# facebookresearch/SlowFast

Measured on AMD Instinct MI355X. Metric: clips/sec (fwd+bwd), SlowFast-8x8-R50 32x224^2 synthetic clips, per-GPU batch 32, higher is better.
Workload: dtype fp16; 1 GPU; SLOWFAST_8x8_R50: forward + cross_entropy loss + backward + sgd step, inputs resident in HBM, per-GPU batch 32; global_batch=32, parallelism=dp1, launch=hip-graph(fwd+bwd) + eager all-reduce/optimizer, optimizer=FlatOptimizer (fused unscale+norm+clip+update, dynamic loss scale on device)

## Files before the change

### slowfast_amd/csrc/sf_api.hip

```cpp
#include "../../include/sfamd.h"
#include "sf_bn.h"
#include "sf_common.h"
#include "sf_igemm.h"
#include "sf_igemm2.h"
#include "sf_wgrad2.h"
#include "sf_pool.h"
#include "sf_dwconv.h"
#include "sf_dwsweep.h"
#include "sf_dwtemporal.h"
#include "sf_tokens.h"
#include "sf_x3d.h"
#include "sf_stem.h"
#include "sf_attn.h"
#include "sf_roi.h"
#include "sf_optim.h"

#include <stdarg.h>
#include <stdio.h>
#include <stdlib.h>
#include <string.h>

static thread_local char g_err[512] = "";

static int fail(const char* fmt, ...) {
// ... 466 lines not shown
    memset(&p, 0, sizeof(p));
    p.g = gather_fwd(d, x, in_scale, in_shift, in_relu);
    p.M = d->N * d->To * d->Ho * d->Wo;
    int32_t ldf, ldd;
    sf_conv_weight_ld(d, &ldf, &ldd);
    p.wmat = (const f16*)wf; p.ldw = ldf; p.Nout = d->Co;
    p.ksteps = cdiv(p.g.Ktot, 32);
    p.y = (f16*)y; p.ldy = d->ldy;
    p.bias = bias; p.resid = nullptr; p.ldr = 0;
    p.stat_part = stat_part;
    return run_igemm(p, is_pointwise(d), (hipStream_t)stream);
}

extern "C" int sf_conv_fwd_fused(const sf_conv_desc* d, const void* x, const void* wf, const float* bias,
                                 const void* resid, int32_t ldr, int out_relu, void* y, sf_stream_t stream) {
    if (check_desc(d)) return -1;
    REQUIRE(x && wf && y, "sf_conv_fwd_fused: null pointer");
    REQUIRE(!resid || (ldr >= d->Co && ldr % 8 == 0), "sf_conv_fwd_fused: bad residual pitch");
    if (!resid) {
        const StemPlan sp = plan_stem(d);
        if (sp.ok) {
            StemParams q = stem_params(d, sp, x);
            int32_t ldf0, ldd0;
            sf_conv_weight_ld(d, &ldf0, &ldd0);
            q.wmat = (const f16*)wf; q.ldw = ldf0; q.y = (f16*)y;
            q.bias = bias; q.out_relu = out_relu;
            SF_STEM_FWD_LAUNCH(sp, q, stream);
            return check_launch("stem_fwd_fused");
        }
    }
    IgemmParams p;
    memset(&p, 0, sizeof(p));
    p.g = gather_fwd(d, x, nullptr, nullptr, 0);
    p.M = d->N * d->To * d->Ho * d->Wo;
    int32_t ldf, ldd;
    sf_conv_weight_ld(d, &ldf, &ldd);
    p.wmat = (const f16*)wf; p.ldw = ldf; p.Nout = d->Co;
    p.ksteps = cdiv(p.g.Ktot, 32);
    p.y = (f16*)y; p.ldy = d->ldy;
    p.bias = bias; p.resid = (const f16*)resid; p.ldr = ldr;
    p.act_mode = out_relu ? 3 : 0;
    return run_igemm(p, is_pointwise(d), (hipStream_t)stream);
}

struct BnFuse {
    const float* scale; const float* shift; const void* bits;
    const void* y0; int32_t ld0; float* part0;
};
static int conv_dgrad_impl(const sf_conv_desc* d, const void* dy, const void* wd, const void* resid, int32_t ldr,
                           const void* resid_bits, void* dx, const BnFuse* bn, int32_t* bn_rows, sf_stream_t stream) {
    if (check_desc(d)) return -1;
    REQUIRE(dy && wd && dx, "sf_conv_dgrad: null pointer");
    REQUIRE(!resid || (ldr >= d->Ci && ldr % 8 == 0), "sf_conv_dgrad: bad residual pitch");
    IgemmParams p;
    memset(&p, 0, sizeof(p));
    p.g = gather_dgrad(d, dy);
    p.M = d->N * d->Ti * d->Hi * d->Wi;
    int32_t ldf, ldd;
    sf_conv_weight_ld(d, &ldf, &ldd);
    p.wmat = (const f16*)wd; p.ldw = ldd; p.Nout = d->Ci;
    p.ksteps = cdiv(p.g.Ktot, 32);
    p.y = (f16*)dx; p.ldy = d->ldx;
    p.resid = (const f16*)resid; p.ldr = ldr;
    REQUIRE(!resid_bits || resid, "sf_conv_dgrad: resid_bits without a residual");
    p.resid_bits = (const uint8_t*)resid_bits;
    const bool fuse = bn && d->sT == 1 && d->sH == 1 && d->sW == 1;
    if (!resid && d->Co == 8 && d->To == d->Ti && d->Ho == d->Hi && d->Wo == d->Wi) {
        sf_conv_desc dd = *d;
        dd.Ci = d->Co; dd.Cw = d->Co; dd.Co = d->Ci; dd.Cow = 0;
        dd.pT = d->kT - 1 - d->pT; dd.pH = d->kH - 1 - d->pH; dd.pW = d->kW - 1 - d->pW;
        dd.ldx = d->ldy; dd.ldy = d->ldx;
        const StemPlan sp = plan_stem(&dd);
        if (sp.ok && sp.thin3 && (!fuse || sp.ntiles <= cdiv(p.M, 128))) {
            StemParams q = stem_params(&dd, sp, dy);
            const int S = d->kT * d->kH;
            q.wmat = (const f16*)wd; q.ldw = ldd; q.y = (f16*)dx;
            q.wo0 = ((S - 1) * 3 + 2) * 8; q.wos = -24; q.wog = -8; q.kwc = 3;
            if (fuse) {
                q.bnb_y = (const f16*)bn->y0; q.bnb_ld = bn->ld0; q.bnb_scale = bn->scale; q.bnb_shift = bn->shift;
                q.bnb_bits = (const uint8_t*)bn->bits;
                q.stat_part = bn->part0; q.stat_rows = 0;
            }
            SF_STEM_FWD_LAUNCH(sp, q, stream);
            if (bn_rows) *bn_rows = fuse ? sp.ntiles : 0;
            return check_launch("stem_dgrad");
        }
    }
    if (fuse) {
        p.bnb_y = (const f16*)bn->y0; p.bnb_ld = bn->ld0; p.bnb_part = bn->part0;
        p.bnb_scale = bn->scale; p.bnb_shift = bn->shift; p.bnb_bits = (const uint8_t*)bn->bits;
    }
    int bm = 0;
    const int rc = run_igemm(p, is_pointwise(d), (hipStream_t)stream, &bm);
    if (bn_rows) *bn_rows = (fuse && bm > 0) ? cdiv(p.M, bm) : 0;
    return rc;
}

extern "C" int sf_conv_dgrad(const sf_conv_desc* d, const void* dy, const void* wd, const void* resid, int32_t ldr,
                             const void* resid_bits, void* dx, sf_stream_t stream) {
    return conv_dgrad_impl(d, dy, wd, resid, ldr, resid_bits, dx, nullptr, nullptr, stream);
}

extern "C" int sf_conv_dgrad_bn(const sf_conv_desc* d, const void* dy, const void* wd, const void* resid, int32_t ldr,
                                const void* resid_bits, void* dx, const float* mask_scale, const float* mask_shift,
                                const void* mask_bits, const void* bn_y, int32_t bn_ldy, float* bn_part, int32_t bn_part_rows,
                                int32_t* bn_rows, sf_stream_t stream) {
    REQUIRE(d && bn_y && bn_part && bn_rows, "sf_conv_dgrad_bn: null pointer");
    REQUIRE(mask_bits || (mask_scale && mask_shift), "sf_conv_dgrad_bn: a mask source is needed (mask_bits, or mask_scale + mask_shift)");
    REQUIRE(bn_ldy >= d->Ci && bn_ldy % 8 == 0 && ((uintptr_t)bn_y & 15) == 0, "sf_conv_dgrad_bn: bad bn_y pitch / alignment");
    REQUIRE((int64_t)bn_part_rows * 128 >= (int64_t)d->N * d->Ti * d->Hi * d->Wi,
            "sf_conv_dgrad_bn: the partial table needs ceil(positions / 128) rows of [2][Ci] floats");
    const BnFuse bn = {mask_scale, mask_shift, mask_bits, bn_y, bn_ldy, bn_part};
    return conv_dgrad_impl(d, dy, wd, resid, ldr, resid_bits, dx, &bn, bn_rows, stream);
}

template <int BMW, int WM, int WN, int KS>
static void launch_wgrad(WgradParams& p, dim3 grid3, hipStream_t s) {
    p.tiles_k = grid3.x; p.tiles_c = grid3.y;
    const dim3 grid(grid3.x * grid3.y * grid3.z);
    hipLaunchKernelGGL((sf_wgrad_kernel<BMW, WM, WN, KS>), grid, dim3(SF_THREADS), 0, s, p);
}

struct WgradPlan {
    int BMW, KS, tiles_k, tiles_c, Co_pad, Kpad, nchunks, chunks_per_split, splits;
    size_t ws_bytes;
};
static WgradPlan plan_wgrad(const sf_conv_desc* d) {
    WgradPlan w;
    const int taps = d->kT * d->kH * d->kW;
    const int Ktot = taps * d->Ci;
    const int64_t M = (int64_t)d->N * d->To * d->Ho * d->Wo;
    w.BMW = d->Co >= 128 ? 128 : d->Co >= 64 ? 64 : d->Co >= 32 ? 32 : 16;
    w.KS = w.BMW <= 32 ? 4 : 1;
    w.tiles_k = cdiv(Ktot, 128);
    w.tiles_c = cdiv(d->Co, w.BMW);
    w.Kpad = w.tiles_k * 128;
    w.Co_pad = w.tiles_c * w.BMW;
    w.nchunks = cdiv(M, 32);
    const int64_t slab = (int64_t)w.Co_pad * w.Kpad * 4;
    static const int target = tune_knob("SF_WGRAD_BLOCKS", 1024);
    int splits = cdiv(target, (int64_t)w.tiles_k * w.tiles_c);
    const int64_t cap = (256ll << 20) / slab;
    if (splits > cap) splits = (int)(cap < 1 ? 1 : cap);
    const int nstages = cdiv(w.nchunks, w.KS);
    if (splits > nstages) splits = nstages;
    if (splits < 1) splits = 1;
    w.chunks_per_split = cdiv(nstages, splits) * w.KS;
    w.splits = cdiv(w.nchunks, w.chunks_per_split);
    w.ws_bytes = (size_t)slab * w.splits;
    return w;
}

struct Wgrad2Plan {
    bool ok, thin, dual;
    int BMW, BKW, tiles_k, tiles_c, Co_pad, Kpad, rows_per_split, splits;
    int slabs;
    size_t tab_bytes, ws_bytes;
};
static Wgrad2Plan plan_wgrad2(const sf_conv_desc* d) {
    Wgrad2Plan w;
    memset(&w, 0, sizeof(w));
    const char* e;
    if (test_hook("SF_WGRAD2", 1) == 0) return w;
    const int mink = test_hook("SF_WGRAD2_MINK", 192);
    const int minrows = test_hook("SF_WGRAD2_MINROWS", 4096);
    const int taps = d->kT * d->kH * d->kW;
    const int target = test_hook("SF_WGRAD2_BLOCKS", 512);
    (void)taps;
    const int Ktot = taps * d->Ci;
    const int64_t M = (int64_t)d->N * d->To * d->Ho * d->Wo;
    if (taps > SF_I2_MAXTAPS || M < minrows) return w;
    if ((d->kT - 1) * d->dT > 127 || (d->kH - 1) * d->dH > 127 || (d->kW - 1) * d->dW > 127) return w;
    if (plan_stem(d).ok) return w;
    if (d->Co <= 32) {
        if (test_hook("SF_WGRAD2T", 1) == 0) return w;
        const int minrows_t = test_hook("SF_WGRAD2T_MINROWS", 16384);
        if (M < minrows_t) return w;
        w.thin = true;
        w.BMW = d->Co <= 16 ? 16 : 32;
        w.BKW = Ktot <= 32 ? 32 : 128;
        w.tiles_k = cdiv(Ktot, w.BKW);
        w.tiles_c = 1;
        w.Kpad = w.tiles_k * w.BKW;
        w.Co_pad = w.BMW;
        const int target_t = test_hook("SF_WGRAD2T_BLOCKS", w.BKW == 128 ? 512 : w.BMW == 32 ? 768 : 1024);
        int splits = target_t / w.tiles_k;
        if (splits < 1) splits = 1;
        w.rows_per_split = roundup(cdiv(M, splits), 128);
        w.splits = cdiv(M, w.rows_per_split);
        w.tab_bytes = ((size_t)M * 8 + 255) / 256 * 256 + 1280;
        w.ws_bytes = w.tab_bytes + (size_t)w.Co_pad * w.Kpad * 4 * w.splits;
        w.slabs = w.splits;
        w.ok = true;
        return w;
    }
    if (Ktot < mink) return w;
    w.BMW = d->Co > 64 ? 128 : 64;
    w.tiles_k = cdiv(Ktot, 256);
    w.tiles_c = cdiv(d->Co, w.BMW);
    w.Kpad = w.tiles_k * 256;
    w.Co_pad = w.tiles_c * w.BMW;
    int splits = target / (w.tiles_k * w.tiles_c);
    const int64_t slab = (int64_t)w.Co_pad * w.Kpad * 4;
    const int64_t cap = (256ll << 20) / slab;
    if (splits > cap) splits = (int)(cap < 1 ? 1 : cap);
    if (splits < 1) splits = 1;
    w.dual = false;
    if (splits >= 2 && test_hook("SF_WGRAD2_DUAL", 1) != 0) {
        const int tiles = w.tiles_k * w.tiles_c;
        const int pairs = (target / 2) / tiles;
        const int64_t steps = cdiv(cdiv(M, splits), 32);
        if (pairs >= 1 && 2 * pairs * 10 >= (2 * pairs < splits ? splits : 2 * pairs) * 9 && steps <= test_hook("SF_WGRAD2_DUAL_STEPS", 80)) {
            w.dual = true;
            if (2 * pairs < splits) splits = 2 * pairs;
        }
    }
    w.rows_per_split = roundup(cdiv(M, splits), 32);
    w.splits = cdiv(M, w.rows_per_split);
    if (w.splits < 2) w.dual = false;
    w.slabs = w.dual ? cdiv(w.splits, 2) : w.splits;
    w.tab_bytes = ((size_t)M * 8 + 255) / 256 * 256 + 1280;
    w.ws_bytes = w.tab_bytes + (size_t)slab * w.splits;
    w.ok = true;
    return w;
}

static void launch_rowtab(const sf_conv_desc* d, void* tab, hipStream_t s) {
    RowtabParams t;
    memset(&t, 0, sizeof(t));
    t.tab = (i32x2*)tab;
    t.M = d->N * d->To * d->Ho * d->Wo;
    t.fdW = make_fastdiv(d->Wo); t.fdH = make_fastdiv(d->Ho); t.fdT = make_fastdiv(d->To);
    t.sT = d->Ti; t.sH = d->Hi; t.sW = d->Wi;
    t.strT = d->sT; t.strH = d->sH; t.strW = d->sW; t.padT = d->pT; t.padH = d->pH; t.padW = d->pW;
    t.ntaps = d->kT * d->kH * d->kW;
    int ti = 0;
    for (int kt = 0; kt < d->kT; ++kt)
        for (int kh = 0; kh < d->kH; ++kh)
            for (int kw = 0; kw < d->kW; ++kw, ++ti) {
                t.dt[ti] = (int8_t)(kt * d->dT); t.dh[ti] = (int8_t)(kh * d->dH); t.dw[ti] = (int8_t)(kw * d->dW);
            }
    hipLaunchKernelGGL(sf_wgrad2_rowtab_kernel, dim3(cdiv(t.M, SF_THREADS)), dim3(SF_THREADS), 0, s, t);
}

extern "C" int64_t sf_conv_wgrad_rowtab_bytes(const sf_conv_desc* d) {
    if (check_desc(d)) return -1;
    const Wgrad2Plan w2 = plan_wgrad2(d);
    return w2.ok ? (int64_t)w2.tab_bytes : 0;
}

extern "C" int sf_conv_wgrad_rowtab(const sf_conv_desc* d, void* tab, sf_stream_t stream) {
    if (check_desc(d)) return -1;
    REQUIRE(tab && (uintptr_t)tab % 16 == 0, "sf_conv_wgrad_rowtab: tab must be a 16-byte aligned device pointer");
    REQUIRE(plan_wgrad2(d).ok, "sf_conv_wgrad_rowtab: this geometry does not take the row-table kernel (sf_conv_wgrad_rowtab_bytes == 0)");
    launch_rowtab(d, tab, (hipStream_t)stream);
    return check_launch("wgrad_rowtab");
}

extern "C" int64_t sf_conv_wgrad_workspace(const sf_conv_desc* d) {
    if (check_desc(d)) return -1;
    int64_t generic = (int64_t)plan_wgrad(d).ws_bytes;
    const Wgrad2Plan w2 = plan_wgrad2(d);
    if (w2.ok && (int64_t)w2.ws_bytes > generic) generic = (int64_t)w2.ws_bytes;
    const StemPlan sp = plan_stem(d);
    return sp.ok && (int64_t)sp.ws_bytes > generic ? (int64_t)sp.ws_bytes : generic;
}

extern "C" int sf_conv_wgrad(const sf_conv_desc* d, const void* x, const float* in_scale, const float* in_shift,
                             int in_relu, const void* dy, float* dw, float out_scale, int zero_first,
                             void* workspace, int64_t workspace_bytes, const void* rowtab, sf_stream_t stream) {
    if (check_desc(d)) return -1;
    REQUIRE(x && dy && dw && workspace, "sf_conv_wgrad: null pointer");
    REQUIRE((in_scale == nullptr) == (in_shift == nullptr), "sf_conv_wgrad: in_scale/in_shift must come together");
    REQUIRE(!in_scale || d->Ci <= 512, "sf_conv_wgrad: fused input BatchNorm supports Ci <= 512 (got %d)", d->Ci);
    hipStream_t s = (hipStream_t)stream;
    int splits, Co_pad, Kpad;
    GatherSide gk = gather_fwd(d, x, in_scale, in_shift, in_relu);
    const StemPlan sp = plan_stem(d);
    const Wgrad2Plan w2 = in_scale ? Wgrad2Plan{} : plan_wgrad2(d);
    float* slabs = (float*)workspace;
    if (w2.ok) {
        REQUIRE(workspace_bytes >= (int64_t)w2.ws_bytes, "sf_conv_wgrad: workspace too small (%lld < %lld bytes)",
                (long long)workspace_bytes, (long long)w2.ws_bytes);
        REQUIRE(((uintptr_t)x | (uintptr_t)dy | (uintptr_t)workspace) % 16 == 0, "sf_conv_wgrad: operands must be 16-byte aligned");
        Wgrad2Params q;
        memset(&q, 0, sizeof(q));
        int ti = 0;
        for (int kt = 0; kt < d->kT; ++kt)
            for (int kh = 0; kh < d->kH; ++kh)
                for (int kw = 0; kw < d->kW; ++kw, ++ti) q.dlin[ti] = (kt * d->dT * d->Hi + kh * d->dH) * d->Wi + kw * d->dW;
        if (!rowtab) launch_rowtab(d, workspace, s);
        else REQUIRE((uintptr_t)rowtab % 16 == 0, "sf_conv_wgrad: rowtab must be 16-byte aligned");
        q.x = (const f16*)x; q.ldx = d->ldx; q.C = d->Ci;
        q.dy = (const f16*)dy; q.ldy = d->ldy; q.Co = d->Co;
        q.M = d->N * d->To * d->Ho * d->Wo; q.Ktot = gk.Ktot;
        q.rowtab = (const i32x2*)(rowtab ? rowtab : workspace);
        slabs = (float*)((char*)workspace + w2.tab_bytes);
        q.ws = slabs; q.Co_pad = w2.Co_pad; q.Kpad = w2.Kpad;
        q.tiles_k = w2.tiles_k; q.tiles_c = w2.tiles_c; q.rows_per_split = w2.rows_per_split;
        q.stage_stride = (w2.thin && tune_knob("SF_WGRAD2T_RR", 1) != 0) ? w2.splits : 0;
        const dim3 grid((unsigned)(w2.tiles_k * w2.tiles_c * w2.slabs));
        static const bool trace = test_hook("SF_TRACE", 0) != 0;
        if (trace) fprintf(stderr, "[sfamd] wgrad2: M=%d Co=%d K=%d tiles %dx%d splits %d%s\n", q.M, q.Co, q.Ktot, w2.tiles_c, w2.tiles_k, w2.splits,
                           w2.dual ? " (two per workgroup)" : "");
        if (w2.thin) {
            if (w2.BMW == 16 && w2.BKW == 128) hipLaunchKernelGGL((sf_wgrad2t_kernel<16, 128, 2>), grid, dim3(256), 0, s, q);
            else if (w2.BMW == 32 && w2.BKW == 128) hipLaunchKernelGGL((sf_wgrad2t_kernel<32, 128, 2>), grid, dim3(256), 0, s, q);
            else if (w2.BMW == 16) hipLaunchKernelGGL((sf_wgrad2t_kernel<16, 32, 3>), grid, dim3(256), 0, s, q);
            else hipLaunchKernelGGL((sf_wgrad2t_kernel<32, 32, 3>), grid, dim3(256), 0, s, q);
        } else if (w2.dual) {
            if (w2.BMW == 128) hipLaunchKernelGGL((sf_wgrad2_kernel<128, true>), grid, dim3(1024), 0, s, q);
            else hipLaunchKernelGGL((sf_wgrad2_kernel<64, true>), grid, dim3(1024), 0, s, q);
        } else {
            if (w2.BMW == 128) hipLaunchKernelGGL((sf_wgrad2_kernel<128>), grid, dim3(512), 0, s, q);
            else hipLaunchKernelGGL((sf_wgrad2_kernel<64>), grid, dim3(512), 0, s, q);
        }
        splits = w2.slabs; Co_pad = w2.Co_pad; Kpad = w2.Kpad;
    } else if (sp.ok && !in_scale) {
        REQUIRE(workspace_bytes >= (int64_t)sp.ws_bytes, "sf_conv_wgrad: workspace too small (%lld < %lld bytes)",
                (long long)workspace_bytes, (long long)sp.ws_bytes);
        StemParams q = stem_params(d, sp, x);
        q.dy = (const f16*)dy; q.ws = (float*)workspace;
        const bool trace = test_hook("SF_TRACE", 0) != 0;
        if (trace) fprintf(stderr, "[sfamd] stem_wgrad: %d workgroups x %d tiles\n", sp.wg_blocks, sp.tiles_per_block);
        static const bool stem_plain = tune_knob("SF_STEM_XCD", 1) == 0;
        q.plain_order = stem_plain ? 1 : 0;
        if (d->Co <= 8 && sp.small) hipLaunchKernelGGL((sf_stem_wgrad_kernel<8, SF_STEM_CHUNKS_SMALL>), dim3(sp.wg_blocks), dim3(SF_STEM_WG_THREADS), 0, s, q);
        else if (d->Co <= 8) hipLaunchKernelGGL((sf_stem_wgrad_kernel<8, SF_STEM_CHUNKS>), dim3(sp.wg_blocks), dim3(SF_STEM_WG_THREADS), 0, s, q);
        else if (sp.small) hipLaunchKernelGGL((sf_stem_wgrad_kernel<16, SF_STEM_CHUNKS_SMALL>), dim3(sp.wg_blocks), dim3(SF_STEM_WG_THREADS), 0, s, q);
        else hipLaunchKernelGGL((sf_stem_wgrad_kernel<16, SF_STEM_CHUNKS>), dim3(sp.wg_blocks), dim3(SF_STEM_WG_THREADS), 0, s, q);
        splits = sp.wg_blocks * sp.wgroups; Co_pad = 16; Kpad = sp.Kpad;
    } else {
        const WgradPlan w = plan_wgrad(d);
        REQUIRE(workspace_bytes >= (int64_t)w.ws_bytes, "sf_conv_wgrad: workspace too small (%lld < %lld bytes)",
                (long long)workspace_bytes, (long long)w.ws_bytes);
        REQUIRE(w.splits <= 65535, "sf_conv_wgrad: too many splits");
        WgradParams p;
        memset(&p, 0, sizeof(p));
        p.g = gk;
        p.dy = (const f16*)dy; p.ldy = d->ldy; p.Co = d->Co;
        p.M = d->N * d->To * d->Ho * d->Wo;
        p.ws = (float*)workspace; p.Co_pad = w.Co_pad; p.Kpad = w.Kpad;
        p.nchunks = w.nchunks; p.chunks_per_split = w.chunks_per_split;
        dim3 grid(w.tiles_k, w.tiles_c, w.splits);
        switch (w.BMW) {
            case 128: launch_wgrad<128, 64, 64, 1>(p, grid, s); break;
            case 64: launch_wgrad<64, 32, 64, 1>(p, grid, s); break;
            case 32: launch_wgrad<32, 32, 32, 4>(p, grid, s); break;
            default: launch_wgrad<16, 16, 32, 4>(p, grid, s); break;
        }
        splits = w.splits; Co_pad = w.Co_pad; Kpad = w.Kpad;
    }
    if (check_launch("wgrad")) return -1;
    WgradReduceParams r;
    r.ws = slabs; r.splits = splits; r.Co = d->Cow ? d->Cow : d->Co; r.Co_pad = Co_pad; r.Kpad = Kpad;
    r.Ktot = gk.Ktot; r.fdC = gk.fdC; r.dw = dw; r.Cw = d->Cw; r.taps = d->kT * d->kH * d->kW;
    r.slice4 = 0;
    if (sp.ok && sp.thin3 && !in_scale && !w2.ok) { r.slice4 = 1; r.Ktot = d->kT * d->kH * 32; }
    r.out_scale = out_scale; r.accumulate = zero_first ? 0 : 1;
    int64_t total = (int64_t)r.Co * Kpad / 4;
    int lanes = 1;
    while (lanes < 32 && lanes * 4 <= splits) lanes *= 2;
    r.lanes = lanes;
    const int per_block = SF_THREADS / lanes;
    hipLaunchKernelGGL(sf_wgrad_reduce_kernel, dim3(cdiv(total, per_block)), dim3(SF_THREADS), 0, s, r);
    return check_launch("wgrad_reduce");
}

static RowTile make_rowtile(int64_t M, int C, int max_blocks, dim3& grid) {
    RowTile rt;
    rt.M = (int)M; rt.C = C;
    const int G = C / 8;
    const int TG = G < SF_THREADS ? G : SF_THREADS;
    const int rpi = SF_THREADS / TG;
    int passes = cdiv(M, (int64_t)rpi * max_blocks);
    if (passes < 1) passes = 1;
    rt.rows_per_block = rpi * passes;
    grid = dim3(cdiv(M, rt.rows_per_block), cdiv(G, SF_THREADS));
    return rt;
}
static int check_rows(const char* who, int64_t M, int C) {
    REQUIRE(M > 0 && M < (1ll << 31), "%s: bad row count", who);
    REQUIRE(C > 0 && C % 8 == 0, "%s: C must be a positive multiple of 8 (got %d)", who, C);
    return 0;
}

static const int kFoldAbove = tune_knob("SF_FOLD_ABOVE", 2048);
static int fold_partials(float* part, int& nblk, int C, hipStream_t s) {
    if (nblk <= kFoldAbove || nblk <= 256) return 1;
    const int group = nblk <= 2048 ? 16 : nblk <= 8192 ? 32 : 64;
    const int cols = 2 * C;
    dim3 grid(cdiv(cols, SF_THREADS), cdiv(nblk, group));
    hipLaunchKernelGGL(sf_part_fold_kernel, grid, dim3(SF_THREADS), 0, s, part, nblk, cols, group);
    nblk = cdiv(nblk, group);
    return group;
}

extern "C" int sf_bn_finalize(float* part, int32_t nblk, int32_t C, int32_t Creal, float count, const float* gamma,
                              const float* beta, float* running_mean, float* running_var, float momentum, float eps,
                              float* scale, float* shift, float* save_mean, float* save_rstd, sf_stream_t stream) {
    REQUIRE(gamma && beta && scale && shift, "sf_bn_finalize: null pointer");
    REQUIRE(nblk > 0 ? part != nullptr : (running_mean && running_var), "sf_bn_finalize: missing statistics source");
    REQUIRE(Creal > 0 && Creal <= C, "sf_bn_finalize: Creal must be in (0, C]");
    BnFinalizeParams p;
    p.row_stride = nblk > 0 ? fold_partials(part, nblk, C, (hipStream_t)stream) : 1;
    p.part = part; p.nblk = nblk; p.C = C; p.Creal = Creal; p.count = count; p.gamma = gamma; p.beta = beta;
    p.running_mean = running_mean; p.running_var = running_var; p.momentum = momentum; p.eps = eps;
    p.scale = scale; p.shift = shift; p.save_mean = save_mean; p.save_rstd = save_rstd;
    hipLaunchKernelGGL(sf_bn_finalize_kernel, dim3(cdiv(C, SF_FIN_CH)), dim3(sf_fin_threads(p.nblk)), 0, (hipStream_t)stream, p);
    return check_launch("bn_finalize");
}

extern "C" int sf_bn_act(int64_t M, int32_t C, const void* y, int32_t ldy, const float* scale, const float* shift,
                         const void* r, int32_t ldr, const float* rscale, const float* rshift, int relu, void* out,
                         int32_t ldo, void* mask_out, sf_stream_t stream) {
    if (check_rows("sf_bn_act", M, C)) return -1;
    REQUIRE(y && out, "sf_bn_act: null pointer");
    BnActParams p;
    dim3 grid;
    p.rt = make_rowtile(M, C, 8192, grid);
    p.y = (const f16*)y; p.ldy = ldy; p.scale = scale; p.shift = shift;
    p.r = (const f16*)r; p.ldr = ldr; p.rscale = rscale; p.rshift = rshift;
    p.relu = relu; p.out = (f16*)out; p.ldo = ldo; p.mask_out = (uint8_t*)mask_out;
    hipLaunchKernelGGL(sf_bn_act_kernel, grid, dim3(SF_THREADS), 0, (hipStream_t)stream, p);
    return check_launch("bn_act");
}

static const int kBwdBlocks = tune_knob("SF_BN_BWD_BLOCKS", 1024);
extern "C" int sf_bn_bwd_blocks(int64_t M, int32_t C) {
    if (check_rows("sf_bn_bwd_blocks", M, C)) return -1;
    dim3 grid;
    make_rowtile(M, C, kBwdBlocks, grid);
    return (int)grid.x;
}

extern "C" int sf_bn_bwd_reduce(int64_t M, int32_t C, const void* dz, int32_t lddz, const void* zmask, int32_t ldm,
                                const void* y, int32_t ldy, const float* scale, const float* shift, int relu_self,
                                float* part, sf_stream_t stream) {
    if (check_rows("sf_bn_bwd_reduce", M, C)) return -1;
    REQUIRE(dz && y && part, "sf_bn_bwd_reduce: null pointer");
    REQUIRE(!relu_self || (scale && shift), "sf_bn_bwd_reduce: relu_self needs scale/shift");
    BnBwdReduceParams p;
    dim3 grid;
    p.rt = make_rowtile(M, C, kBwdBlocks, grid);
    p.dz = (const f16*)dz; p.lddz = lddz; p.zmask = (const f16*)zmask; p.ldm = ldm;
    p.y = (const f16*)y; p.ldy = ldy; p.scale = scale; p.shift = shift; p.relu_self = relu_self; p.part = part;
    hipLaunchKernelGGL(sf_bn_bwd_reduce_kernel, grid, dim3(SF_THREADS), 0, (hipStream_t)stream, p);
    return check_launch("bn_bwd_reduce");
}

extern "C" int sf_bn_bwd_finalize(float* part, int32_t nblk, int32_t C, int32_t Creal, float count, const float* gamma,
                                  const float* mean, const float* rstd, float inv_loss_scale, float* dgamma,
                                  float* dbeta, int accumulate, float* coef, sf_stream_t stream) {
    REQUIRE(part && gamma && mean && rstd && dgamma && dbeta && coef, "sf_bn_bwd_finalize: null pointer");
    BnBwdFinalizeParams p;
    p.row_stride = fold_partials(part, nblk, C, (hipStream_t)stream);
    REQUIRE(Creal > 0 && Creal <= C, "sf_bn_bwd_finalize: Creal must be in (0, C]");
    p.part = part; p.nblk = nblk; p.C = C; p.Creal = Creal; p.count = count; p.gamma = gamma; p.mean = mean; p.rstd = rstd;
    p.inv_loss_scale = inv_loss_scale; p.dgamma = dgamma; p.dbeta = dbeta; p.accumulate = accumulate; p.coef = coef;
    hipLaunchKernelGGL(sf_bn_bwd_finalize_kernel, dim3(cdiv(C, SF_FIN_CH)), dim3(sf_fin_threads(p.nblk)), 0, (hipStream_t)stream, p);
    return check_launch("bn_bwd_finalize");
}
// ... 1632 lines not shown
```

### slowfast_amd/csrc/sf_wgrad2.h

```cpp
#pragma once
#include "sf_common.h"
#include "sf_igemm2.h"

struct __attribute__((aligned(8))) i32x2 { int32_t x, y; };
typedef int32_t i32x8 __attribute__((ext_vector_type(8)));

struct Wgrad2Params {
    const f16* x; int ldx, C;
    const f16* dy; int ldy, Co;
    int M;
    int Ktot;
    const i32x2* rowtab;
    int32_t dlin[SF_I2_MAXTAPS];
    float* ws;
    int Co_pad, Kpad;
    int tiles_k, tiles_c;
    int rows_per_split;
    int stage_stride;
};

struct RowtabParams {
    i32x2* tab;
    int M;
    FastDiv fdW, fdH, fdT;
    int sT, sH, sW;
    int strT, strH, strW, padT, padH, padW;
    int ntaps;
    int8_t dt[SF_I2_MAXTAPS], dh[SF_I2_MAXTAPS], dw[SF_I2_MAXTAPS];
};

__global__ __launch_bounds__(SF_THREADS) void sf_wgrad2_rowtab_kernel(RowtabParams p) {
    const int m = blockIdx.x * SF_THREADS + threadIdx.x;
    if (m >= p.M) return;
    uint32_t q, a, b, c, n;
    fd_divmod((uint32_t)m, p.fdW, q, c);
    fd_divmod(q, p.fdH, q, b);
    fd_divmod(q, p.fdT, n, a);
    const int bt = (int)a * p.strT - p.padT, bh = (int)b * p.strH - p.padH, bw = (int)c * p.strW - p.padW;
    uint32_t mk = 0;
    for (int t = 0; t < p.ntaps; ++t) {
        const int st = bt + p.dt[t], sh = bh + p.dh[t], sw = bw + p.dw[t];
        const bool ok = (unsigned)st < (unsigned)p.sT && (unsigned)sh < (unsigned)p.sH && (unsigned)sw < (unsigned)p.sW;
        mk |= (ok ? 1u : 0u) << t;
    }
    i32x2 e;
    e.x = (((int)n * p.sT + bt) * p.sH + bh) * p.sW + bw;
    e.y = (int)mk;
    p.tab[m] = e;
}

__device__ __forceinline__ int w2_swz(int m) { return (m & 3) | (((m >> 3) & 1) << 2); }

template <int BMW, bool DUAL = false>
__global__ __launch_bounds__(DUAL ? 1024 : 512, 4) void sf_wgrad2_kernel(Wgrad2Params p) {
    constexpr int BKW = 256, ROWS = 32, NW = 8, NST = 3;
    constexpr int WAVES_C = BMW / 64, WAVES_K = NW / WAVES_C;
    constexpr int WN = BKW / WAVES_K;
    constexpr int TM = 4, TN = WN / 16;
    constexpr int Y_ELEMS = ROWS * BMW, X_ELEMS = ROWS * BKW, STAGE = Y_ELEMS + X_ELEMS;
    constexpr int YI = Y_ELEMS / 512;
    constexpr int YRPI = 512 / BMW;
    constexpr int YCH = BMW / 8;
    __shared__ __attribute__((aligned(16))) f16 smem_all[(DUAL ? 2 : 1) * NST * STAGE];

    const int tid = threadIdx.x;
    const int lane = tid & 63, wave_all = __builtin_amdgcn_readfirstlane(tid >> 6);
    const int half = DUAL ? wave_all >> 3 : 0, wave = wave_all & 7;
    f16* const smem = smem_all + half * (NST * STAGE);
    const int wc = wave / WAVES_K, wk = wave % WAVES_K;
    const uint32_t wg = xcd_remap(blockIdx.x, gridDim.x);
    const int bx = (int)(wg % (uint32_t)p.tiles_k);
    const int by = (int)((wg / (uint32_t)p.tiles_k) % (uint32_t)p.tiles_c);
    const int bz = (int)(wg / ((uint32_t)p.tiles_k * (uint32_t)p.tiles_c));
    const int k0 = bx * BKW, c0 = by * BMW;
    const int r0 = (DUAL ? 2 * bz + half : bz) * p.rows_per_split;
    int r1 = r0 + p.rows_per_split;
    if (r1 > p.M) r1 = p.M;
    const int nsteps = r1 > r0 ? (r1 - r0 + ROWS - 1) / ROWS : 0;
    int nsteps_wg = nsteps;
    if constexpr (DUAL) {
        const int ra = 2 * bz * p.rows_per_split;
        int rb = ra + p.rows_per_split;
        if (rb > p.M) rb = p.M;
        nsteps_wg = rb > ra ? (rb - ra + ROWS - 1) / ROWS : 0;
    }
    const f16* const zline = reinterpret_cast<const f16*>(sf_zero_line);

    const int xrr = lane >> 5, xpc = lane & 31;
    int64_t xcol[2];
    uint32_t xbit[2];
#pragma unroll
    for (int j = 0; j < 2; ++j) {
        const int mrow = 2 * (wave + 8 * j) + xrr;
        const int lchunk = (((xpc >> 1) ^ w2_swz(mrow)) << 1) | (xpc & 1);
        const int k = k0 + lchunk * 8;
        if (k < p.Ktot) {
            const int tap = k / p.C, ci = k - tap * p.C;
            xbit[j] = 1u << tap;
            xcol[j] = (int64_t)p.dlin[tap] * p.ldx + ci;
        } else {
            xbit[j] = 0u;
            xcol[j] = 0;
        }
    }
    const int yrr = lane / YCH, ypc = lane % YCH;
    const bool ywave = wave < YI;
    const int ymrow = YRPI * wave + yrr;
    int ylchunk;
    if constexpr (BMW == 128) ylchunk = (((ypc >> 1) ^ w2_swz(ymrow)) << 1) | (ypc & 1);
    else ylchunk = (((ypc >> 1) ^ (((ymrow >> 1) & 1) | (((ymrow >> 3) & 1) << 1))) << 1) | (ypc & 1);
    const int yco = c0 + ylchunk * 8;
    const bool yok = yco < p.Co;

    auto tab_rows = [&](int step, i32x2 (&e)[2][2]) {
#pragma unroll
        for (int j = 0; j < 2; ++j)
#pragma unroll
            for (int r = 0; r < 2; ++r) {
                const int m = r0 + step * ROWS + 2 * (wave + 8 * j) + r;
                i32x2 v;
                v.x = 0; v.y = 0;
                if (m < r1) {
                    v.x = SF_SCALAR_PTR(i32x2, p.rowtab)[m].x;
                    v.y = SF_SCALAR_PTR(i32x2, p.rowtab)[m].y;
                }
                e[j][r] = v;
            }
    };
    auto issue = [&](int step, int buf, const i32x2 (&e)[2][2]) {
        f16* Ys = smem + buf * STAGE;
        f16* Xs = Ys + Y_ELEMS;
        if (ywave) {
            const int m = r0 + step * ROWS + ymrow;
            const f16* g = (m < r1 && yok) ? p.dy + (int64_t)m * p.ldy + yco : zline;
            SF_GLOBAL_LOAD_LDS16_ASM(g, Ys + wave * 512);
        }
#pragma unroll
        for (int j = 0; j < 2; ++j) {
            const int pos = xrr ? e[j][1].x : e[j][0].x;
            const uint32_t mk = (uint32_t)(xrr ? e[j][1].y : e[j][0].y);
            const bool ok = (mk & xbit[j]) != 0u;
            const f16* g = ok ? p.x + ((int64_t)pos * p.ldx + xcol[j]) : zline;
            SF_GLOBAL_LOAD_LDS16_ASM(g, Xs + (wave + 8 * j) * 512);
        }
    };

    f32x4 acc[TM][TN];
#pragma unroll
    for (int i = 0; i < TM; ++i)
#pragma unroll
        for (int j = 0; j < TN; ++j) acc[i][j] = (f32x4){0.f, 0.f, 0.f, 0.f};

    const int pl = lane & 15, g4 = lane >> 4;
    auto compute = [&](int buf) {
        const f16* Ys = smem + buf * STAGE;
        const f16* Xs = Ys + Y_ELEMS;
        f16x8 af[TM], bf[TN];
#pragma unroll
        for (int h = 0; h < 2; ++h) {
            const int m = 8 * g4 + 4 * h + (pl >> 2);
#pragma unroll
            for (int i = 0; i < TM; ++i) {
                const int col = wc * 64 + i * 16;
                int off;
                if constexpr (BMW == 128) off = m * BMW + ((((col >> 4) ^ w2_swz(m)) << 4) | (4 * (pl & 3)));
                else off = m * BMW + ((((col >> 4) ^ (((m >> 1) & 1) | (((m >> 3) & 1) << 1))) << 4) | (4 * (pl & 3)));
                const f16x4 t = as_f16x4(SF_LDS_TR16(Ys + off));
                af[i][4 * h + 0] = t[0]; af[i][4 * h + 1] = t[1]; af[i][4 * h + 2] = t[2]; af[i][4 * h + 3] = t[3];
            }
#pragma unroll
            for (int j = 0; j < TN; ++j) {
                const int col = wk * WN + j * 16;
                const int off = m * BKW + ((((col >> 4) ^ w2_swz(m)) << 4) | (4 * (pl & 3)));
                const f16x4 t = as_f16x4(SF_LDS_TR16(Xs + off));
                bf[j][4 * h + 0] = t[0]; bf[j][4 * h + 1] = t[1]; bf[j][4 * h + 2] = t[2]; bf[j][4 * h + 3] = t[3];
            }
        }
#pragma unroll
        for (int i = 0; i < TM; ++i)
#pragma unroll
            for (int j = 0; j < TN; ++j)
                acc[i][j] = SF_MFMA16(af[i], bf[j], acc[i][j]);
    };

    {
        constexpr int COPIES = 2;
        i32x2 e[2][2];
        int issued = 0;
        for (; issued < NST - 1 && issued < nsteps; ++issued) { tab_rows(issued, e); issue(issued, issued, e); }
        if (issued < nsteps) tab_rows(issued, e);
        int cur = 0, nxt = NST - 1;
        for (int ks = 0; ks < nsteps_wg; ++ks) {
            if (ks + NST - 2 < nsteps) {
                SF_WAIT_VMEM_N(COPIES);
            } else SF_WAIT_VMEM();
            SF_BARRIER_KEEP_VMEM();
            if (issued < nsteps) {
                issue(issued, nxt, e);
                ++issued;
                if (issued < nsteps) tab_rows(issued, e);
            }
            if (!DUAL || ks < nsteps) compute(cur);
            cur = cur == NST - 1 ? 0 : cur + 1;
            nxt = nxt == NST - 1 ? 0 : nxt + 1;
        }
    }

    constexpr int I0 = 0, IH = DUAL ? TM / 2 : TM;
    if constexpr (DUAL) {
        static_assert(TM % 2 == 0, "the halves split the fragment rows");
        static_assert(2 * NST * STAGE * 2 >= 2 * IH * TN * 4 * 512 * 4, "the exchange reuses both rings");
        __syncthreads();
        float* xch = reinterpret_cast<float*>(smem_all);
        const int t512 = tid & 511;
        float* mine = xch + half * (IH * TN * 4 * 512);
        const float* theirs = xch + (1 - half) * (IH * TN * 4 * 512);
#pragma unroll
        for (int ii = 0; ii < IH; ++ii)
#pragma unroll
            for (int j = 0; j < TN; ++j)
#pragma unroll
                for (int r = 0; r < 4; ++r) {
                    const f32x4& a0 = acc[ii][j];
                    const f32x4& a1 = acc[IH + ii][j];
                    mine[((ii * TN + j) * 4 + r) * 512 + t512] = half ? a0[r] : a1[r];
                }
        __syncthreads();
#pragma unroll
        for (int ii = 0; ii < IH; ++ii)
#pragma unroll
            for (int j = 0; j < TN; ++j)
#pragma unroll
                for (int r = 0; r < 4; ++r) {
                    const float o = theirs[((ii * TN + j) * 4 + r) * 512 + t512];
                    if (half) acc[IH + ii][j][r] += o; else acc[ii][j][r] += o;
                }
    }

    float* slab = p.ws + (int64_t)bz * p.Co_pad * p.Kpad;
#pragma unroll
    for (int j = 0; j < TN; ++j) {
        const int kcol = k0 + wk * WN + j * 16 + pl;
#pragma unroll
        for (int ii = I0; ii < IH; ++ii)
#pragma unroll
            for (int r = 0; r < 4; ++r) {
                if constexpr (DUAL) {
                    const int co0 = c0 + wc * 64 + ii * 16 + 4 * g4 + r;
                    const float v0 = acc[ii][j][r], v1 = acc[IH + ii][j][r];
                    slab[(int64_t)(co0 + (half ? IH * 16 : 0)) * p.Kpad + kcol] = half ? v1 : v0;
                } else {
                    const int co = c0 + wc * 64 + ii * 16 + 4 * g4 + r;
                    slab[(int64_t)co * p.Kpad + kcol] = acc[ii][j][r];
                }
            }
    }
}

__device__ __forceinline__ int w2t_swap23(int m) { return (m & ~12) | ((m & 4) << 1) | ((m & 8) >> 1); }
template <int W>
__device__ __forceinline__ int w2t_frag_off(int m, int tile) {
    if constexpr (W == 128) return m * 128 + ((tile ^ w2_swz(m)) << 4);
    else if constexpr (W == 32) return m * 32 + ((tile ^ ((m >> 3) & 1)) << 4);
    else return w2t_swap23(m) * 16;
}
template <int W>
__device__ __forceinline__ void w2t_slot(int prow, int pc, int& row, int& chunk) {
    if constexpr (W == 128) { row = prow; chunk = (((pc >> 1) ^ w2_swz(prow)) << 1) | (pc & 1); }
    else if constexpr (W == 32) { row = prow; chunk = (((pc >> 1) ^ ((prow >> 3) & 1)) << 1) | (pc & 1); }
    else { row = w2t_swap23(prow); chunk = pc; }
}

template <int BMW, int BKW, int NST>
__global__ __launch_bounds__(256) void sf_wgrad2t_kernel(Wgrad2Params p) {
    constexpr int ROWS = 128, NW = 4;
    constexpr int TMC = BMW / 16, TNK = BKW / 16;
    constexpr int YCH = BMW / 8, XCH = BKW / 8;
    constexpr int YRPI = 64 / YCH, XRPI = 64 / XCH;
    constexpr int YPW = ROWS / YRPI / NW, XPW = ROWS / XRPI / NW;
    constexpr int COPIES = YPW + XPW;
    constexpr int Y_ELEMS = ROWS * BMW, X_ELEMS = ROWS * BKW, STAGE = Y_ELEMS + X_ELEMS;
    static_assert(NST * STAGE * 2 >= NW * TMC * TNK * 256 * 4, "the cross-wave reduction reuses the stage buffers");
    __shared__ __attribute__((aligned(16))) f16 smem[NST * STAGE];

    const int tid = threadIdx.x;
    const int lane = tid & 63, wave = __builtin_amdgcn_readfirstlane(tid >> 6);
    const uint32_t wg = xcd_remap(blockIdx.x, gridDim.x);
    const int bx = (int)(wg % (uint32_t)p.tiles_k);
    const int bz = (int)(wg / (uint32_t)p.tiles_k);
    const int k0 = bx * BKW;
    const int rr = p.stage_stride > 0;
    const int r0 = rr ? bz * ROWS : bz * p.rows_per_split;
    const int rstep = rr ? p.stage_stride * ROWS : ROWS;
    int r1 = rr ? p.M : r0 + p.rows_per_split;
    if (r1 > p.M) r1 = p.M;
    const int nsteps = r1 > r0 ? (r1 - r0 + rstep - 1) / rstep : 0;
    const f16* const zline = reinterpret_cast<const f16*>(sf_zero_line);

    int xrow[XPW];
    int xsel[XPW];
    int64_t xcol[XPW];
    uint32_t xbit[XPW];
#pragma unroll
    for (int j = 0; j < XPW; ++j) {
        const int q = wave + NW * j;
        int row, chunk;
        w2t_slot<BKW>(q * XRPI + lane / XCH, lane % XCH, row, chunk);
        xrow[j] = row;
        xsel[j] = row - q * XRPI;
        const int k = k0 + chunk * 8;
        if (k < p.Ktot) {
            const int tap = k / p.C, ci = k - tap * p.C;
            xbit[j] = 1u << tap;
            xcol[j] = (int64_t)p.dlin[tap] * p.ldx + ci;
        } else {
            xbit[j] = 0u;
            xcol[j] = 0;
        }
    }
    int yrow[YPW];
    int yco[YPW];
#pragma unroll
    for (int j = 0; j < YPW; ++j) {
        const int q = wave + NW * j;
        int row, chunk;
        w2t_slot<BMW>(q * YRPI + lane / YCH, lane % YCH, row, chunk);
        yrow[j] = row;
        yco[j] = chunk * 8;
    }

    auto tab_rows = [&](int step, int (&epos)[XPW], uint32_t (&emk)[XPW]) {
        i32x8 t[XPW][XRPI / 4];
#pragma unroll
        for (int j = 0; j < XPW; ++j) {
            const int m0 = r0 + step * rstep + (wave + NW * j) * XRPI;
#pragma unroll
            for (int r = 0; r < XRPI / 4; ++r) t[j][r] = SF_SCALAR_PTR(i32x8, p.rowtab + m0)[r];
        }
#pragma unroll
        for (int j = 0; j < XPW; ++j) {
            const int m0 = r0 + step * rstep + (wave + NW * j) * XRPI;
            int pos = 0;
            uint32_t mk = 0u;
#pragma unroll
            for (int r = 0; r < XRPI; ++r)
                if (xsel[j] == r) { pos = t[j][r / 4][2 * (r % 4)]; mk = (uint32_t)t[j][r / 4][2 * (r % 4) + 1]; }
            epos[j] = pos;
            emk[j] = (m0 + xsel[j] < r1) ? mk : 0u;
        }
    };
    auto issue = [&](int step, int buf, const int (&epos)[XPW], const uint32_t (&emk)[XPW]) {
        f16* Ys = smem + buf * STAGE;
        f16* Xs = Ys + Y_ELEMS;
#pragma unroll
        for (int j = 0; j < YPW; ++j) {
            const int m = r0 + step * rstep + yrow[j];
            const f16* g = (m < r1 && yco[j] < p.Co) ? p.dy + (int64_t)m * p.ldy + yco[j] : zline;
            SF_GLOBAL_LOAD_LDS16_ASM(g, Ys + (wave + NW * j) * 512);
        }
#pragma unroll
        for (int j = 0; j < XPW; ++j) {
            const bool ok = (emk[j] & xbit[j]) != 0u;
            const f16* g = ok ? p.x + ((int64_t)epos[j] * p.ldx + xcol[j]) : zline;
            SF_GLOBAL_LOAD_LDS16_ASM(g, Xs + (wave + NW * j) * 512);
        }
    };

    f32x4 acc[TMC][TNK];
#pragma unroll
    for (int i = 0; i < TMC; ++i)
#pragma unroll
        for (int j = 0; j < TNK; ++j) acc[i][j] = (f32x4){0.f, 0.f, 0.f, 0.f};

    const int pl = lane & 15, g4 = lane >> 4;
    auto compute = [&](int buf) {
        const f16* Ys = smem + buf * STAGE;
        const f16* Xs = Ys + Y_ELEMS;
        f16x8 af[TMC], bf[TNK];
#pragma unroll
        for (int h = 0; h < 2; ++h) {
            const int m = wave * 32 + 8 * g4 + 4 * h + (pl >> 2);
#pragma unroll
            for (int i = 0; i < TMC; ++i) {
                const f16x4 t = as_f16x4(SF_LDS_TR16(Ys + w2t_frag_off<BMW>(m, i) + 4 * (pl & 3)));
                af[i][4 * h + 0] = t[0]; af[i][4 * h + 1] = t[1]; af[i][4 * h + 2] = t[2]; af[i][4 * h + 3] = t[3];
            }
#pragma unroll
            for (int j = 0; j < TNK; ++j) {
                const f16x4 t = as_f16x4(SF_LDS_TR16(Xs + w2t_frag_off<BKW>(m, j) + 4 * (pl & 3)));
                bf[j][4 * h + 0] = t[0]; bf[j][4 * h + 1] = t[1]; bf[j][4 * h + 2] = t[2]; bf[j][4 * h + 3] = t[3];
            }
        }
// ... 50 lines not shown
```

Before: 871.2 clips/s.

## Add transposed wgrad2 path for 1x1 convs with small Ci and wide Co

Adds a SWAP variant of the wgrad2 kernel for pointwise convolutions where Ci<=128. The roles of x and dy are swapped so the wide operand (dy, Co channels) fills the 256-wide K tile and the narrow Ci sits in the BMW tile. Slabs are written with vectorized f32x4 stores in the transposed layout. The aim is to cut padding waste and get better tile utilization on shapes that were previously rejected (Ktot < mink) or poorly tiled. The cost is another kernel instantiation and different split heuristics.

```diff
diff --git a/slowfast_amd/csrc/sf_api.hip b/slowfast_amd/csrc/sf_api.hip
--- a/slowfast_amd/csrc/sf_api.hip
+++ b/slowfast_amd/csrc/sf_api.hip
@@ -642,7 +642,7 @@
 }
 
 struct Wgrad2Plan {
-    bool ok, thin, dual;
+    bool ok, thin, dual, swap;
     int BMW, BKW, tiles_k, tiles_c, Co_pad, Kpad, rows_per_split, splits;
     int slabs;
     size_t tab_bytes, ws_bytes;
@@ -684,12 +684,25 @@
         w.ok = true;
         return w;
     }
-    if (Ktot < mink) return w;
-    w.BMW = d->Co > 64 ? 128 : 64;
-    w.tiles_k = cdiv(Ktot, 256);
-    w.tiles_c = cdiv(d->Co, w.BMW);
-    w.Kpad = w.tiles_k * 256;
-    w.Co_pad = w.tiles_c * w.BMW;
+    if (const int sw = test_hook("SF_WGRAD2_SWAP", 1); sw != 0 && taps == 1 && Ktot <= 128) {
+        const int bmw = Ktot <= 64 ? 64 : 128;
+        const int co_pad = roundup(d->Co, 256);
+        w.swap = sw == 2 || (Ktot * 4 >= bmw * 3 && d->Co * 4 >= co_pad * 3);
+    }
+    if (!w.swap && Ktot < mink) return w;
+    if (w.swap) {
+        w.BMW = Ktot <= 64 ? 64 : 128;
+        w.tiles_k = cdiv(d->Co, 256);
+        w.tiles_c = 1;
+        w.Kpad = w.BMW;
+        w.Co_pad = w.tiles_k * 256;
+    } else {
+        w.BMW = d->Co > 64 ? 128 : 64;
+        w.tiles_k = cdiv(Ktot, 256);
+        w.tiles_c = cdiv(d->Co, w.BMW);
+        w.Kpad = w.tiles_k * 256;
+        w.Co_pad = w.tiles_c * w.BMW;
+    }
     int splits = target / (w.tiles_k * w.tiles_c);
     const int64_t slab = (int64_t)w.Co_pad * w.Kpad * 4;
     const int64_t cap = (256ll << 20) / slab;
@@ -791,13 +804,18 @@
         q.stage_stride = (w2.thin && tune_knob("SF_WGRAD2T_RR", 1) != 0) ? w2.splits : 0;
         const dim3 grid((unsigned)(w2.tiles_k * w2.tiles_c * w2.slabs));
         static const bool trace = test_hook("SF_TRACE", 0) != 0;
-        if (trace) fprintf(stderr, "[sfamd] wgrad2: M=%d Co=%d K=%d tiles %dx%d splits %d%s\n", q.M, q.Co, q.Ktot, w2.tiles_c, w2.tiles_k, w2.splits,
-                           w2.dual ? " (two per workgroup)" : "");
+        if (trace) fprintf(stderr, "[sfamd] wgrad2: M=%d Co=%d K=%d tiles %dx%d splits %d%s%s\n", q.M, q.Co, q.Ktot, w2.tiles_c, w2.tiles_k, w2.splits,
+                           w2.dual ? " (two per workgroup)" : "", w2.swap ? " (transposed)" : "");
         if (w2.thin) {
             if (w2.BMW == 16 && w2.BKW == 128) hipLaunchKernelGGL((sf_wgrad2t_kernel<16, 128, 2>), grid, dim3(256), 0, s, q);
             else if (w2.BMW == 32 && w2.BKW == 128) hipLaunchKernelGGL((sf_wgrad2t_kernel<32, 128, 2>), grid, dim3(256), 0, s, q);
             else if (w2.BMW == 16) hipLaunchKernelGGL((sf_wgrad2t_kernel<16, 32, 3>), grid, dim3(256), 0, s, q);
             else hipLaunchKernelGGL((sf_wgrad2t_kernel<32, 32, 3>), grid, dim3(256), 0, s, q);
+        } else if (w2.swap) {
+            if (w2.dual && w2.BMW == 128) hipLaunchKernelGGL((sf_wgrad2_kernel<128, true, true>), grid, dim3(1024), 0, s, q);
+            else if (w2.dual) hipLaunchKernelGGL((sf_wgrad2_kernel<64, true, true>), grid, dim3(1024), 0, s, q);
+            else if (w2.BMW == 128) hipLaunchKernelGGL((sf_wgrad2_kernel<128, false, true>), grid, dim3(512), 0, s, q);
+            else hipLaunchKernelGGL((sf_wgrad2_kernel<64, false, true>), grid, dim3(512), 0, s, q);
         } else if (w2.dual) {
             if (w2.BMW == 128) hipLaunchKernelGGL((sf_wgrad2_kernel<128, true>), grid, dim3(1024), 0, s, q);
             else hipLaunchKernelGGL((sf_wgrad2_kernel<64, true>), grid, dim3(1024), 0, s, q);
diff --git a/slowfast_amd/csrc/sf_wgrad2.h b/slowfast_amd/csrc/sf_wgrad2.h
--- a/slowfast_amd/csrc/sf_wgrad2.h
+++ b/slowfast_amd/csrc/sf_wgrad2.h
@@ -51,7 +51,7 @@
 
 __device__ __forceinline__ int w2_swz(int m) { return (m & 3) | (((m >> 3) & 1) << 2); }
 
-template <int BMW, bool DUAL = false>
+template <int BMW, bool DUAL = false, bool SWAP = false>
 __global__ __launch_bounds__(DUAL ? 1024 : 512, 4) void sf_wgrad2_kernel(Wgrad2Params p) {
     constexpr int BKW = 256, ROWS = 32, NW = 8, NST = 3;
     constexpr int WAVES_C = BMW / 64, WAVES_K = NW / WAVES_C;
@@ -94,7 +94,10 @@
         const int mrow = 2 * (wave + 8 * j) + xrr;
         const int lchunk = (((xpc >> 1) ^ w2_swz(mrow)) << 1) | (xpc & 1);
         const int k = k0 + lchunk * 8;
-        if (k < p.Ktot) {
+        if constexpr (SWAP) {
+            xbit[j] = k < p.Co ? 1u : 0u;
+            xcol[j] = k < p.Co ? k : 0;
+        } else if (k < p.Ktot) {
             const int tap = k / p.C, ci = k - tap * p.C;
             xbit[j] = 1u << tap;
             xcol[j] = (int64_t)p.dlin[tap] * p.ldx + ci;
@@ -110,7 +113,7 @@
     if constexpr (BMW == 128) ylchunk = (((ypc >> 1) ^ w2_swz(ymrow)) << 1) | (ypc & 1);
     else ylchunk = (((ypc >> 1) ^ (((ymrow >> 1) & 1) | (((ymrow >> 3) & 1) << 1))) << 1) | (ypc & 1);
     const int yco = c0 + ylchunk * 8;
-    const bool yok = yco < p.Co;
+    const bool yok = yco < (SWAP ? p.Ktot : p.Co);
 
     auto tab_rows = [&](int step, i32x2 (&e)[2][2]) {
 #pragma unroll
@@ -120,27 +123,48 @@
                 const int m = r0 + step * ROWS + 2 * (wave + 8 * j) + r;
                 i32x2 v;
                 v.x = 0; v.y = 0;
-                if (m < r1) {
+                if constexpr (SWAP) {
+                    v.x = m; v.y = m < r1 ? 1 : 0;
+                } else if (m < r1) {
                     v.x = SF_SCALAR_PTR(i32x2, p.rowtab)[m].x;
                     v.y = SF_SCALAR_PTR(i32x2, p.rowtab)[m].y;
                 }
                 e[j][r] = v;
             }
     };
-    auto issue = [&](int step, int buf, const i32x2 (&e)[2][2]) {
+    auto ytab_row = [&](int step, i32x2& ye) {
+        ye.x = 0; ye.y = 0;
+        if constexpr (SWAP) {
+            if (ywave) {
+                const int m0 = r0 + step * ROWS + YRPI * wave;
+                i32x8 t[YRPI / 4];
+#pragma unroll
+                for (int r = 0; r < YRPI / 4; ++r) t[r] = SF_SCALAR_PTR(i32x8, p.rowtab + m0)[r];
+#pragma unroll
+                for (int r = 0; r < YRPI; ++r)
+                    if (yrr == r) { ye.x = t[r / 4][2 * (r % 4)]; ye.y = t[r / 4][2 * (r % 4) + 1]; }
+                if (m0 + yrr >= r1) ye.y = 0;
+            }
+        }
+    };
+    auto issue = [&](int step, int buf, const i32x2 (&e)[2][2], const i32x2& ye) {
         f16* Ys = smem + buf * STAGE;
         f16* Xs = Ys + Y_ELEMS;
         if (ywave) {
             const int m = r0 + step * ROWS + ymrow;
-            const f16* g = (m < r1 && yok) ? p.dy + (int64_t)m * p.ldy + yco : zline;
+            const f16* g;
+            if constexpr (SWAP) g = ((ye.y & 1) && yok) ? p.x + ((int64_t)ye.x * p.ldx + yco) : zline;
+            else g = (m < r1 && yok) ? p.dy + (int64_t)m * p.ldy + yco : zline;
             SF_GLOBAL_LOAD_LDS16_ASM(g, Ys + wave * 512);
         }
+        const f16* const wide = SWAP ? p.dy : p.x;
+        const int ldwide = SWAP ? p.ldy : p.ldx;
 #pragma unroll
         for (int j = 0; j < 2; ++j) {
             const int pos = xrr ? e[j][1].x : e[j][0].x;
             const uint32_t mk = (uint32_t)(xrr ? e[j][1].y : e[j][0].y);
             const bool ok = (mk & xbit[j]) != 0u;
-            const f16* g = ok ? p.x + ((int64_t)pos * p.ldx + xcol[j]) : zline;
+            const f16* g = ok ? wide + ((int64_t)pos * ldwide + xcol[j]) : zline;
             SF_GLOBAL_LOAD_LDS16_ASM(g, Xs + (wave + 8 * j) * 512);
         }
     };
@@ -185,10 +209,10 @@
 
     {
         constexpr int COPIES = 2;
-        i32x2 e[2][2];
+        i32x2 e[2][2], ye;
         int issued = 0;
-        for (; issued < NST - 1 && issued < nsteps; ++issued) { tab_rows(issued, e); issue(issued, issued, e); }
-        if (issued < nsteps) tab_rows(issued, e);
+        for (; issued < NST - 1 && issued < nsteps; ++issued) { tab_rows(issued, e); ytab_row(issued, ye); issue(issued, issued, e, ye); }
+        if (issued < nsteps) { tab_rows(issued, e); ytab_row(issued, ye); }
         int cur = 0, nxt = NST - 1;
         for (int ks = 0; ks < nsteps_wg; ++ks) {
             if (ks + NST - 2 < nsteps) {
@@ -196,9 +220,9 @@
             } else SF_WAIT_VMEM();
             SF_BARRIER_KEEP_VMEM();
             if (issued < nsteps) {
-                issue(issued, nxt, e);
+                issue(issued, nxt, e, ye);
                 ++issued;
-                if (issued < nsteps) tab_rows(issued, e);
+                if (issued < nsteps) { tab_rows(issued, e); ytab_row(issued, ye); }
             }
             if (!DUAL || ks < nsteps) compute(cur);
             cur = cur == NST - 1 ? 0 : cur + 1;
@@ -238,6 +262,22 @@
     }
 
     float* slab = p.ws + (int64_t)bz * p.Co_pad * p.Kpad;
+    if constexpr (SWAP) {
+#pragma unroll
+        for (int j = 0; j < TN; ++j) {
+            const int co = k0 + wk * WN + j * 16 + pl;
+#pragma unroll
+            for (int ii = I0; ii < IH; ++ii) {
+                f32x4 v = acc[ii][j];
+                int i = ii;
+                if constexpr (DUAL) {
+                    if (half) { v = acc[IH + ii][j]; i = IH + ii; }
+                }
+                *reinterpret_cast<f32x4*>(slab + (int64_t)co * p.Kpad + (c0 + wc * 64 + i * 16 + 4 * g4)) = v;
+            }
+        }
+        return;
+    }
 #pragma unroll
     for (int j = 0; j < TN; ++j) {
         const int kcol = k0 + wk * WN + j * 16 + pl;
```

Result: no change. 873.2 clips/s (median of 6 runs) (+0.2%).
